# Meng-333/SRADSGAN

Hardware: AMD Instinct MI355X
Metric: training images/sec (216x216, x4) (higher is better)
Workload: dtype f32 (split-bf16 products: 3 bf16 MFMA terms per fp32 multiply, fp32 accumulate)

## Files before the change

sradsgan_amd/csrc/conv_api.hip:

```cpp
#include "conv_internal.h"
#include "conv_dev.h"

using namespace srhip;

namespace srhip {
struct PackEntry {
  const float* w;
  float* packed;
  int cout, cin, kh, kw, mode, fast;
};
__global__ __launch_bounds__(256) void pack_batched_kernel(const PackEntry* __restrict__ tab) {
  const PackEntry e = tab[blockIdx.y];
  const int khkw = e.kh * e.kw;
  if (e.fast) {
    constexpr int LDS_F = 32 * (16 * 9 + 1);
    __shared__ float tile[LDS_F];
    const long total = (long)e.cout * e.cin * khkw;
    const int RO = e.mode == 0 ? 8 : 32;
    const int CI = e.mode == 0 ? (khkw <= 9 ? 64 : 16) : (khkw <= 9 ? 16 : 4);
    const int ld = CI * khkw + 1;
    const int nci = (e.cin + CI - 1) / CI, nco = (e.cout + RO - 1) / RO;
    const int ndst = e.mode == 0 ? e.cout : e.cin, csrc = e.mode == 0 ? e.cin : e.cout;
    const long ndst16 = ((long)ndst + 15) / 16 * 16;
    float* s0 = e.packed;
// ... 5 lines not shown
      const int cw = min(CI, e.cin - ci0), rw = min(RO, e.cout - co0);
      const int rowlen = cw * khkw;
      __syncthreads();
      for (int i = threadIdx.x; i < rw * rowlen; i += 256) {
        const int r = i / rowlen, k = i - r * rowlen;
        tile[r * ld + k] = e.w[((size_t)(co0 + r) * e.cin + ci0) * khkw + k];
      }
      __syncthreads();
      auto at = [&](int a, int b, int tap) { return tile[a * ld + b * khkw + tap]; };
      const int nn = e.mode == 0 ? rw : cw, nc = e.mode == 0 ? cw : rw;
      const int n0 = e.mode == 0 ? co0 : ci0, c00 = e.mode == 0 ? ci0 : co0;
      for (int it = threadIdx.x; it < nn * khkw * (nc / 8); it += 256) {
        const int g8 = it % (nc / 8), rt = it / (nc / 8);
        const int tap = rt % khkw, dn = rt / khkw;
        float v[8];
#pragma unroll
        for (int j = 0; j < 8; ++j) v[j] = e.mode == 0 ? at(dn, g8 * 8 + j, tap) : at(g8 * 8 + j, dn, tap);
        const long idx = ((long)(n0 + dn) * khkw + tap) * csrc + c00 + g8 * 8;
        reinterpret_cast<float4*>(s0 + idx)[0] = make_float4(v[0], v[1], v[2], v[3]);
        reinterpret_cast<float4*>(s0 + idx)[1] = make_float4(v[4], v[5], v[6], v[7]);
        bf16x8_t hi, lo;
        split_bf16x8(make_float4(v[0], v[1], v[2], v[3]), make_float4(v[4], v[5], v[6], v[7]), hi, lo);
        *reinterpret_cast<u32x4*>(s1 + idx * 4) = __builtin_bit_cast(u32x4, hi);
        *reinterpret_cast<u32x4*>(s1 + idx * 4 + 16) = __builtin_bit_cast(u32x4, lo);
        const f16x8_t f16 = {(_Float16)v[0], (_Float16)v[1], (_Float16)v[2], (_Float16)v[3], (_Float16)v[4], (_Float16)v[5], (_Float16)v[6], (_Float16)v[7]};
        const u32x4 z = {0u, 0u, 0u, 0u};
        *reinterpret_cast<u32x4*>(s2 + idx * 4) = __builtin_bit_cast(u32x4, f16);
        *reinterpret_cast<u32x4*>(s2 + idx * 4 + 16) = z;
      }
      for (int it = threadIdx.x; it < nn * khkw * (nc / 16); it += 256) {
        const int dn = it % nn, rt = it / nn;
        const int tap = rt % khkw, g16 = rt / khkw;
        const int n = n0 + dn, swz = (n >> 2) & 3;
        char* row = s3 + (((long)((c00 >> 4) + g16) * khkw + tap) * ndst16 + n) * 64;
#pragma unroll
        for (int h = 0; h < 2; ++h) {
          float v[8];
#pragma unroll
          for (int j = 0; j < 8; ++j) v[j] = e.mode == 0 ? at(dn, g16 * 16 + h * 8 + j, tap) : at(g16 * 16 + h * 8 + j, dn, tap);
          bf16x8_t hi, lo;
          split_bf16x8(make_float4(v[0], v[1], v[2], v[3]), make_float4(v[4], v[5], v[6], v[7]), hi, lo);
          *reinterpret_cast<u32x4*>(row + (((2 * h) ^ swz) << 4)) = __builtin_bit_cast(u32x4, hi);
          *reinterpret_cast<u32x4*>(row + (((2 * h + 1) ^ swz) << 4)) = __builtin_bit_cast(u32x4, lo);
        }
      }
    }
  } else {
    const int csrc = e.mode == 0 ? e.cin : e.cout, cdst = e.mode == 0 ? e.cout : e.cin;
    const int ld = ((cdst + 31) / 32) * 32;
    const long total = (long)khkw * csrc * ld;
    for (long idx = (long)blockIdx.x * blockDim.x + threadIdx.x; idx < total; idx += (long)gridDim.x * blockDim.x) {
      const int row = (int)(idx / ld), col = (int)(idx - (long)row * ld);
      float v = 0.f;
      if (col < cdst) {
        const int tap = row / csrc, cs = row - tap * csrc;
        const int a = tap / e.kw, b = tap - a * e.kw;
        if (e.mode == 0)
          v = e.w[(((size_t)col * e.cin + cs) * e.kh + a) * e.kw + b];
        else
          v = e.w[(((size_t)cs * e.cin + col) * e.kh + (e.kh - 1 - a)) * e.kw + (e.kw - 1 - b)];
      }
      e.packed[idx] = v;
    }
  }
}
}

namespace srhip {
extern int g_fast_cfg;
extern int g_wgrad_cfg;
extern int g_rowtap_addr;
extern int g_rowtap_pipe;
extern int g_patch_ks;
extern int g_fast_dynlds;
extern int g_fast_ablate;
extern int g_conv_math;
extern int g_sgam_cfg;
extern int g_pers_grid;
extern int g_pers_small;
extern int g_pool_epi_any;
extern int g_pers_abl;
extern int g_phase_batch;
extern int g_headconv_rows;
}
extern int g_tail_dbg;
namespace srhip {
}

namespace srhip {
struct Probe {
  int kind = 0, n = 0, h = 0, w = 0, cin = 0, cout = 0, cap = 0, count = 0;
  hipEvent_t ev[2 * 1024];
  int units[1024];
  int created = 0;
};
static Probe g_probe;
static inline bool probe_hit(int kind, int n, int h, int w, int cin, int cout) {
  return g_probe.kind == kind && g_probe.count < g_probe.cap && g_probe.n == n && g_probe.h == h && g_probe.w == w && g_probe.cin == cin &&
         g_probe.cout == cout;
}
static inline int probe_begin(void* stream) {
  const int i = g_probe.count;
  (void)hipEventRecord(g_probe.ev[2 * i], as_stream(stream));
  return i;
}
static inline void probe_end(int i, void* stream, int units = 1) {
  (void)hipEventRecord(g_probe.ev[2 * i + 1], as_stream(stream));
  g_probe.units[i] = units;
  g_probe.count = i + 1;
}
}

extern "C" {

int srhip_probe_config(int kind, int n, int h, int w, int cin, int cout, int max_pairs) {
  SRHIP_REQUIRE(kind >= 0 && kind <= 3 && max_pairs >= 0 && max_pairs <= 1024, "probe_config: kind 0..3, max_pairs <= 1024");
  while (g_probe.created < 2 * max_pairs) {
    if (hipEventCreate(&g_probe.ev[g_probe.created]) != hipSuccess) {
      set_error("probe_config: hipEventCreate failed");
      return SRHIP_ERR_LAUNCH;
    }
    ++g_probe.created;
  }
  g_probe.kind = kind; g_probe.n = n; g_probe.h = h; g_probe.w = w; g_probe.cin = cin; g_probe.cout = cout;
  g_probe.cap = kind ? max_pairs : 0;
  g_probe.count = 0;
  return SRHIP_OK;
}
int srhip_probe_read(float* ms, int* units, int cap) {
  SRHIP_REQUIRE(ms || cap == 0, "probe_read: null buffer");
  const int n = g_probe.count < cap ? g_probe.count : cap;
  for (int i = 0; i < n; ++i) {
    if (hipEventSynchronize(g_probe.ev[2 * i + 1]) != hipSuccess || hipEventElapsedTime(&ms[i], g_probe.ev[2 * i], g_probe.ev[2 * i + 1]) != hipSuccess) {
      set_error("probe_read: event %d not readable", i);
      return -1;
    }
    if (units) units[i] = g_probe.units[i];
  }
  return n;
}

int srhip_debug_set(int key, int value) {
  if (key == 0) {
    g_fast_cfg = value;
    return SRHIP_OK;
  }
  if (key == 1) {
    g_wgrad_cfg = value;
    return SRHIP_OK;
  }
  if (key == 2) {
    g_fast_dynlds = value;
    return SRHIP_OK;
  }
  if (key == 3) {
    g_fast_ablate = value;
    return SRHIP_OK;
  }
  if (key == 4) {
    g_sgam_cfg = value;
    return SRHIP_OK;
  }
  if (key == 5) {
    g_pers_grid = value;
    return SRHIP_OK;
  }
  if (key == 6) {
    g_pers_abl = value;
    return SRHIP_OK;
  }
  if (key == 7) {
    g_tail_dbg = value;
    return SRHIP_OK;
  }
  if (key == 8) {
    g_rowtap_addr = value;
    return SRHIP_OK;
  }
  if (key == 9) {
    g_rowtap_pipe = value;
    return SRHIP_OK;
  }
  if (key == 10) {
    g_patch_ks = value;
    return SRHIP_OK;
  }
  if (key == 11) {
    g_pers_small = value;
    return SRHIP_OK;
  }
  if (key == 12) {
    g_flat_blocks = value > 0 ? value : 768;
    return SRHIP_OK;
  }
  if (key == 13) {
    g_flat_abl = value;
    return SRHIP_OK;
  }
  if (key == 14) {
    g_flat_f32_k8 = value;
    return SRHIP_OK;
  }
  if (key == 15) {
    g_patch8 = value;
    return SRHIP_OK;
  }
  if (key == 16) {
    g_patch8_abl = value;
    return SRHIP_OK;
  }
  if (key == 17) {
    g_phase_batch = value;
    return SRHIP_OK;
  }
  if (key == 18) {
    g_headconv_rows = value;
    return SRHIP_OK;
  }
  if (key == 19) {
    g_pool_epi_any = value;
    return SRHIP_OK;
  }
  return SRHIP_ERR_ARG;
}

int srhip_set_conv_math(int mode) {
  SRHIP_REQUIRE(mode == SRHIP_MATH_FP32 || mode == SRHIP_MATH_BF16X3 || mode == SRHIP_MATH_HALF, "set_conv_math: unknown mode");
  g_conv_math = mode;
  return SRHIP_OK;
}
int srhip_get_conv_math(void) { return g_conv_math; }

size_t srhip_packed_elems(int cout, int cin, int kh, int kw, int mode) {
  if (cout <= 0 || cin <= 0 || kh <= 0 || kw <= 0 || (mode != 0 && mode != 1)) return 0;
  const bool fast = mode == 0 ? fast_fwd_ok(cin, cout, kh, kw) : fast_dgrad_ok(cin, cout, kh, kw);
  if (fast)
    return 3 * (size_t)cout * cin * kh * kw + (size_t)fast_tiled_elems(mode == 0 ? cout : cin, mode == 0 ? cin : cout, kh * kw);
  const int csrc = mode == 0 ? cin : cout, cdst = mode == 0 ? cout : cin;
  return (size_t)kh * kw * csrc * legacy_packed_ld(cdst);
}

int srhip_pack_entry_bytes(void) { return (int)sizeof(PackEntry); }

int srhip_packed_is_fast(int cout, int cin, int kh, int kw, int mode) {
  return (mode == 0 ? fast_fwd_ok(cin, cout, kh, kw) : fast_dgrad_ok(cin, cout, kh, kw)) ? 1 : 0;
}

int srhip_pack_weights_batched(const void* entries_dev, int count, void* stream) {
  SRHIP_REQUIRE(entries_dev && count >= 0, "pack_weights_batched: bad argument");
  if (count == 0) return SRHIP_OK;
  hipLaunchKernelGGL(pack_batched_kernel, dim3(32, count), dim3(256), 0, as_stream(stream),
                     static_cast<const PackEntry*>(entries_dev));
  return check_launch("pack_weights_batched");
}

int srhip_pack_weight(const float* w, float* packed, int cout, int cin, int kh, int kw, int mode, void* stream) {
  SRHIP_REQUIRE(w && packed && cout > 0 && cin > 0 && kh > 0 && kw > 0 && (mode == 0 || mode == 1),
                "pack_weight: bad argument");
  const bool fast = mode == 0 ? fast_fwd_ok(cin, cout, kh, kw) : fast_dgrad_ok(cin, cout, kh, kw);
  if (fast) return fast_pack_weight(w, packed, cout, cin, kh, kw, mode, as_stream(stream));
  return legacy_pack_weight(w, packed, cout, cin, kh, kw, mode, stream);
}

int srhip_conv2d_fwd(const float* x, const float* packed, const float* bias, const float* residual,
                     const float* rowscale, const float* chanscale, float* y, int n, int h, int w, int cin, int cout, int kh, int kw,
                     int stride, int pad, int ldx, int ldy, int ldr, float slope, int flags, void* stream) {
  SRHIP_REQUIRE(x && packed && y, "conv2d_fwd: null tensor");
  SRHIP_REQUIRE(n >= 0 && h > 0 && w > 0 && cin > 0 && cout > 0 && kh > 0 && kw > 0 && stride > 0 && pad >= 0,
                "conv2d_fwd: bad geometry");
  SRHIP_REQUIRE(ldx >= cin && ldy >= cout, "conv2d_fwd: row stride smaller than channel count");
  SRHIP_REQUIRE(!(flags & SRHIP_EPI_BIAS) || bias, "conv2d_fwd: EPI_BIAS without bias");
  SRHIP_REQUIRE(!(flags & SRHIP_EPI_RESIDUAL) || (residual && ldr >= cout), "conv2d_fwd: EPI_RESIDUAL without residual");
  SRHIP_REQUIRE(!(flags & SRHIP_EPI_ROWSCALE) || rowscale, "conv2d_fwd: EPI_ROWSCALE without rowscale");
  SRHIP_REQUIRE(!(flags & SRHIP_EPI_CHANSCALE) || chanscale, "conv2d_fwd: EPI_CHANSCALE without chanscale");
  if (fast_fwd_ok(cin, cout, kh, kw)) {
    const bool pr = probe_hit(1, n, h, w, cin, cout);
    const int pi = pr ? probe_begin(stream) : 0;
    const int rc = fast_conv2d_fwd(x, packed, bias, residual, rowscale, chanscale, y, n, h, w, cin, cout, kh, kw, stride, pad, ldx, ldy,
                                   ldr, slope, flags, as_stream(stream));
    if (pr) probe_end(pi, stream);
    return rc;
  }
  SRHIP_REQUIRE(!(flags & SRHIP_EPI_CHANSCALE), "conv2d_fwd: EPI_CHANSCALE needs Cin % 16 == 0");
  return legacy_conv2d_fwd(x, packed, bias, residual, rowscale, y, n, h, w, cin, cout, kh, kw, stride, pad, ldx, ldy,
                           ldr, slope, flags, stream);
}

int srhip_conv2d_fwd_dual(const float* x, const float* packed, const float* bias, const float* residual, const float* rowscale,
                          const float* chanscale, float* y, void* y_pp, int* served, int n, int h, int w, int cin, int cout, int kh,
                          int kw, int stride, int pad, int ldx, int ldy, int ldr, float slope, int flags, void* stream) {
  SRHIP_REQUIRE(y_pp && served && (((uintptr_t)y_pp) & 15) == 0 && ldy == cout, "conv2d_fwd_dual: 16-byte aligned plane buffer, dense fp32 output");
  g_dst2_req.pp = y_pp;
  g_dst2_req.served = 0;
  const int rc = srhip_conv2d_fwd(x, packed, bias, residual, rowscale, chanscale, y, n, h, w, cin, cout, kh, kw, stride, pad, ldx, ldy, ldr,
                                  slope, flags, stream);
  *served = g_dst2_req.served;
  g_dst2_req.pp = nullptr;
  g_dst2_req.served = 0;
  return rc;
}

int srhip_conv2d_fwd_pool(const float* x, const float* packed, const float* bias, float* y, float* pool, size_t pool_sec_bytes,
                          int* nseg_out, int n, int h, int w, int cin, int cout, int ldx, int ldy, int flags, void* stream) {
// ... 279 lines not shown
```

sradsgan_amd/csrc/conv_fast.hip:

```cpp
#include "conv_dev.h"

namespace srhip {

int g_fast_ablate = 0;



template <int BM, int BN, int WM, int WN, int BK, int MATH = 0>
__global__ __launch_bounds__(WM* WN * 64) void fast_conv_kernel(const float* __restrict__ src,
                                                                 const float* __restrict__ wt,
                                                                 const float* __restrict__ bias,
                                                                 const float* __restrict__ residual,
                                                                 const float* __restrict__ rowscale,
                                                                 const float* __restrict__ chanscale,
                                                                 const float* __restrict__ actmask,
                                                                 float* __restrict__ dst, FastGeom g, int nblk_m,
                                                                 int nblk_n) {
  constexpr int NT = WM * WN * 64;
  constexpr int WTM = BM / WM, WTN = BN / WN;
  constexpr int TM = WTM / 32, TN = WTN / 32;
  constexpr int LS = BK + 4;
  constexpr int QPR = BK / 4;
  constexpr int RPP = NT / QPR;
  constexpr int AR = (BM + RPP - 1) / RPP, BR = (BN + RPP - 1) / RPP;
// ... 1067 lines not shown
template <int ND>
__global__ __launch_bounds__(256) void narrow_conv_kernel(const float* __restrict__ src, const float* __restrict__ wt,
                                                           const float* __restrict__ bias, float* __restrict__ dst,
                                                           FastGeom g, int tiles_h, int tiles_w, int lo_h, int lo_w) {
  constexpr int PW = 16, PH = 16, PWP = PW + 2, PR = (PH + 2) * PWP;
  __shared__ __attribute__((aligned(16))) float4 lds[2][PR * 4];
  const int tid = threadIdx.x;
  const int tpi = tiles_h * tiles_w;
  const int img = blockIdx.x / tpi;
  const int prem = blockIdx.x - img * tpi;
  const int ty = prem / tiles_w, tx = prem - ty * tiles_w;
  const int oh0 = ty * PH, ow0 = tx * PW;
  const int py = tid >> 4, px = tid & 15;

  int soff[6];
  int sdst[6];
#pragma unroll
  for (int i = 0; i < 6; ++i) {
    const int e = tid + i * 256;
    soff[i] = -1;
    sdst[i] = 0;
    if (e < PR * 4) {
      const int row = e >> 2, q = e & 3;
      const int pi = row / PWP, pj = row - pi * PWP;
      const int sh = oh0 + lo_h + pi, sw = ow0 + lo_w + pj;
      sdst[i] = row * 4 + (q ^ (row & 3));
      if (sh >= 0 && sh < g.Hs && sw >= 0 && sw < g.Ws) soff[i] = ((img * g.Hs + sh) * g.Ws + sw) * g.lds + q * 4;
      else soff[i] = -2;
    }
  }
  const int CC = g.C / 16;
  float4 stage[6];
  auto fetch = [&](int cc) {
#pragma unroll
    for (int i = 0; i < 6; ++i)
      stage[i] = soff[i] >= 0 ? *reinterpret_cast<const float4*>(src + (size_t)soff[i] + cc * 16) : make_float4(0.f, 0.f, 0.f, 0.f);
  };
  auto commit = [&](int buf) {
#pragma unroll
    for (int i = 0; i < 6; ++i)
      if (soff[i] != -1) lds[buf][sdst[i]] = stage[i];
  };
  float acc[ND];
#pragma unroll
  for (int n = 0; n < ND; ++n) acc[n] = 0.f;

  fetch(0);
  commit(0);
  __syncthreads();
  for (int cc = 0; cc < CC; ++cc) {
    const int buf = cc & 1;
    if (cc + 1 < CC) fetch(cc + 1);
#pragma unroll 1
    for (int tap = 0; tap < 9; ++tap) {
      {
        const int th = tap / 3, tw = tap - th * 3;
        const int a_th = (g.dh0 + th * g.dhs) - lo_h, a_tw = (g.dw0 + tw * g.dws) - lo_w;
        const int row = (py + a_th) * PWP + px + a_tw;
        const int wk = ((g.kh0 + th * g.khs) * g.KW + (g.kw0 + tw * g.kws)) * g.C + cc * 16;
#pragma unroll
        for (int q = 0; q < 4; ++q) {
          const float4 v = lds[buf][row * 4 + (q ^ (row & 3))];
#pragma unroll
          for (int n = 0; n < ND; ++n) {
            const float* w = wt + (size_t)n * g.ldw + wk + q * 4;
            acc[n] = fmaf(v.x, w[0], acc[n]);
            acc[n] = fmaf(v.y, w[1], acc[n]);
            acc[n] = fmaf(v.z, w[2], acc[n]);
            acc[n] = fmaf(v.w, w[3], acc[n]);
          }
        }
      }
    }
    if (cc + 1 < CC) commit(buf ^ 1);
    __syncthreads();
  }
  const int oh = oh0 + py, ow = ow0 + px;
  if (oh < g.OH && ow < g.OW) {
    const size_t dpix = ((size_t)img * g.Hd + oh) * g.Wd + ow;
#pragma unroll
    for (int n = 0; n < ND; ++n) {
      if (n < g.K) {
        float v = acc[n];
        if (g.flags & SRHIP_EPI_BIAS) v += bias[n];
        if (g.flags & SRHIP_EPI_LRELU) v = v > 0.f ? v : v * g.slope;
        dst[dpix * g.ldd + n] = v;
      }
    }
  }
}

struct WgradGeom {
  int N, H, W, C, ldx;
  int Ho, Wo, K, ldy;
  int KH, KW, stride, pad;
  int P;
  int Ktot;
  int nsplit, chunks_per_split;
  unsigned x_bytes, dy_bytes;
};

template <int BM, int BN, int WM, int WN>
__global__ __launch_bounds__(256) void fast_wgrad_kernel(const float* __restrict__ x, const float* __restrict__ dy,
                                                          float* __restrict__ partial,
                                                          float* __restrict__ bias_partial,
                                                          const float* __restrict__ xrow,
                                                          const float* __restrict__ xchan, WgradGeom g) {
  constexpr int WTM = BM / WM, WTN = BN / WN;
  constexpr int TM = WTM / 32, TN = WTN / 32;
  constexpr int LDA = BM + 4, LDB = BN + 4;
  constexpr int AV = (FBK * BM / 4) / 256, BV = (FBK * BN / 4) / 256;
  static_assert(AV >= 1 && BV >= 1, "tile too small");
  constexpr int STAGE = FBK * (LDA + LDB);
  __shared__ __attribute__((aligned(16))) float lds[2 * STAGE];

  const int tid = threadIdx.x;
  const int ntn = (g.Ktot + BN - 1) / BN;
  const int ntm = (g.K + BM - 1) / BM;
  int tile_n, tile_m, split;
  {
    const int tps = ntm * ntn;
    int bid = blockIdx.x;
    if (g.nsplit % 8 == 0) {
      const int j = bid >> 3;
      split = (j / tps) * 8 + (bid & 7);
      bid = j % tps;
    } else {
      split = bid / tps;
      bid -= split * tps;
    }
    tile_n = bid % ntn;
    tile_m = bid / ntn;
  }
  const int m0 = tile_m * BM, n0 = tile_n * BN;

  __amdgpu_buffer_rsrc_t rx = __builtin_amdgcn_make_buffer_rsrc(const_cast<float*>(x), 0, g.x_bytes, 0x00020000);
  __amdgpu_buffer_rsrc_t ry = __builtin_amdgcn_make_buffer_rsrc(const_cast<float*>(dy), 0, g.dy_bytes, 0x00020000);

  const int c_begin = split * g.chunks_per_split;
  const int nchunks_total = (g.P + FBK - 1) / FBK;
  const int c_end = min(c_begin + g.chunks_per_split, nchunks_total);

  constexpr int AQ = BM / 4, BQ = BN / 4;
  const int a_row0 = tid / AQ, a_c = tid - a_row0 * AQ;
  const int b_row0 = tid / BQ, b_c = tid - b_row0 * BQ;
  const bool a_colok = (m0 + a_c * 4) < g.K;
  const int kcol = n0 + b_c * 4;
  const bool b_colok = kcol < g.Ktot;
  const int tap = kcol / g.C, ci0 = kcol - tap * g.C;
  const int kh = tap / g.KW, kw = tap - kh * g.KW;

  int bn[BV], bho[BV], bwo[BV];
#pragma unroll
  for (int j = 0; j < BV; ++j) {
    const int p = c_begin * FBK + b_row0 + j * (256 / BQ);
    const int HoWo = g.Ho * g.Wo;
    bn[j] = p / HoWo;
    const int rem = p - bn[j] * HoWo;
    bho[j] = rem / g.Wo;
    bwo[j] = rem - bho[j] * g.Wo;
  }

  float4 ra[AV], rb[BV], rxs[BV];
  float4 bsum = make_float4(0.f, 0.f, 0.f, 0.f);
  const bool xscale = xrow != nullptr || xchan != nullptr;
  auto load_tiles = [&](int kc) {
// ... 958 lines not shown
                                 int kw, int mode) {
  const int idx = blockIdx.x * blockDim.x + threadIdx.x;
  const int total = cout * cin * kh * kw;
  if (idx >= total) return;
  const int khkw = kh * kw;
  if (mode == 0) {
    const int co = idx / (khkw * cin);
    const int rem = idx - co * khkw * cin;
    const int tap = rem / cin, ci = rem - tap * cin;
    fast_pack_store(packed, total, idx, w[((size_t)co * cin + ci) * khkw + tap], cout, cin, khkw);
  } else {
    const int ci = idx / (khkw * cout);
    const int rem = idx - ci * khkw * cout;
    const int tap = rem / cout, co = rem - tap * cout;
    fast_pack_store(packed, total, idx, w[((size_t)co * cin + ci) * khkw + tap], cin, cout, khkw);
  }
}

static bool shape_ok(int csrc, int kh, int kw) { return csrc % 16 == 0 && kh * kw <= 32 && kh == kw; }
bool fast_fwd_ok(int cin, int cout, int kh, int kw) { return shape_ok(cin, kh, kw); }
bool fast_dgrad_ok(int cin, int cout, int kh, int kw) { return shape_ok(cout, kh, kw); }
bool fast_wgrad_ok(int cin, int cout, int kh, int kw) { return cin % 16 == 0 && cout % 4 == 0 && kh == kw; }

int fast_pack_weight(const float* w, float* packed, int cout, int cin, int kh, int kw, int mode, hipStream_t st) {
  const long total = (long)cout * cin * kh * kw;
  hipLaunchKernelGGL(fast_pack_kernel, dim3(cdiv(total, 256)), dim3(256), 0, st, w, packed, cout, cin, kh, kw, mode);
  return check_launch("fast_pack_weight");
}

thread_local Dst2Request g_dst2_req;
thread_local ResRequest g_res_req;
thread_local PhaseRequest g_phase_req;
int g_conv_math = 0;
int g_fast_dynlds = 0;
template <int BM, int BN, int WM, int WN, int BK>
static int launch_fast(const float* src, const float* wt, const float* bias, const float* residual,
                       const float* rowscale, const float* chanscale, const float* actmask, float* dst,
                       const FastGeom& g, hipStream_t st) {
  const int nbm = cdiv(g.M, BM), nbn = cdiv(g.K, BN);
  hipLaunchKernelGGL((fast_conv_kernel<BM, BN, WM, WN, BK>), dim3(nbm * nbn), dim3(WM * WN * 64), g_fast_dynlds, st, src, wt, bias,
                     residual, rowscale, chanscale, actmask, dst, g, nbm, nbn);
  return check_launch("fast_conv");
}

__global__ __launch_bounds__(256) void dot_conv_kernel(const float* __restrict__ src, const float* __restrict__ wt,
                                                        const float* __restrict__ bias, float* __restrict__ dst, FastGeom g) {
  const int lane = threadIdx.x & 63;
  const int m = blockIdx.x * 4 + (threadIdx.x >> 6);
  if (m >= g.M) return;
  const int ow = m % g.OW, t = m / g.OW;
  const int oh = t % g.OH, n = t / g.OH;
  float acc = 0.f;
  for (int th = 0; th < g.TH; ++th) {
    const int sh = oh * g.ss + g.dh0 + th * g.dhs;
    if (sh < 0 || sh >= g.Hs) continue;
    for (int tw = 0; tw < g.TW; ++tw) {
      const int sw = ow * g.ss + g.dw0 + tw * g.dws;
      if (sw < 0 || sw >= g.Ws) continue;
      const float* xp = src + ((size_t)(n * g.Hs + sh) * g.Ws + sw) * g.lds;
      const float* wp = wt + (size_t)((g.kh0 + th * g.khs) * g.KW + (g.kw0 + tw * g.kws)) * g.C;
      for (int c = lane * 4; c < g.C; c += 256) {
        const float4 a = *reinterpret_cast<const float4*>(xp + c);
        const float4 b = *reinterpret_cast<const float4*>(wp + c);
        acc = fmaf(a.x, b.x, acc);
        acc = fmaf(a.y, b.y, acc);
        acc = fmaf(a.z, b.z, acc);
        acc = fmaf(a.w, b.w, acc);
      }
    }
  }
#pragma unroll
  for (int o = 32; o >= 1; o >>= 1) acc += __shfl_xor(acc, o, 64);
  if (lane == 0) {
    float v = acc;
    if (g.flags & SRHIP_EPI_BIAS) v += bias[0];
    if (g.flags & SRHIP_EPI_LRELU) v = v > 0.f ? v : v * g.slope;
    dst[((size_t)(n * g.Hd + oh * g.dsd + g.ph) * g.Wd + ow * g.dsd + g.pw) * g.ldd] = v;
  }
}

int g_patch_ks = 1;
int g_fast_cfg = 0;
int g_phase_batch = 1;

static bool plan_patch(const FastGeom& g, PatchGeom* pg, double min_eff = 0.70) {
  if (g.TH != 3 || g.TW != 3 || g.ss != 1 || g.dsd != 1 || g.ph != 0 || g.pw != 0) return false;
  if ((g.dhs != 1 && g.dhs != -1) || (g.dws != 1 && g.dws != -1)) return false;
  if (g.Hd != g.OH || g.Wd != g.OW) return false;
  double best = 0.0;
  for (int pw = 4; pw <= 64 && pw <= g.OW + 3; ++pw) {
    int ph = 128 / pw;
    if (ph > g.OH) ph = g.OH;
    if (ph < 1 || (ph + 2) * (pw + 2) > 192) continue;
    const long tiles = (long)cdiv(g.OH, ph) * cdiv(g.OW, pw);
    const double eff = (double)g.OH * g.OW / ((double)tiles * 128.0) + 1e-6 * (double)(pw - pw % 16) / pw;
    if (eff > best + 1e-9) {
      best = eff;
      pg->PH = ph; pg->PW = pw;
    }
  }
  if (best < min_eff || best <= 0.0) return false;
  pg->tiles_h = cdiv(g.OH, pg->PH);
  pg->tiles_w = cdiv(g.OW, pg->PW);
  pg->PWP = pg->PW + 2;
  pg->PR = (pg->PH + 2) * pg->PWP;
  pg->npieces = cdiv(pg->PR, 16);
  pg->lo_h = g.dhs > 0 ? g.dh0 : g.dh0 + 2 * g.dhs;
  pg->lo_w = g.dws > 0 ? g.dw0 : g.dw0 + 2 * g.dws;
  const int a = pg->PW >> 4;
  const int nfull = pg->PH * a < 8 ? pg->PH * a : 8;
  auto base = [&](int q) { return ((q / a) * pg->PWP + (q % a) * 16) & 15; };
  int fin[8], nf = 0, singles[8], ns = 0;
  bool used[8] = {false, false, false, false, false, false, false, false};
  for (int q = 0; q < nfull; ++q) {
    if (used[q]) continue;
    used[q] = true;
    int partner = -1;
    for (int p2 = q + 1; p2 < nfull; ++p2)
      if (!used[p2] && base(p2) == base(q)) {
        partner = p2;
        break;
      }
    if (partner >= 0) {
      used[partner] = true;
      fin[nf++] = q;
      fin[nf++] = partner;
    } else {
      singles[ns++] = q;
    }
  }
  for (int i = 0; i < ns; ++i) fin[nf++] = singles[i];
  for (int q = nfull; q < 8; ++q) fin[nf++] = q;
  pg->gmap = 0;
  for (int i = 0; i < 8; ++i) pg->gmap |= (unsigned)(fin[i] & 15) << (4 * i);
  return true;
}

long pp_sign_tiles(int n, int h, int w, int cout) {
  if (cout < 128 || cout % 128 != 0) return 0;
  FastGeom g;
  g.TH = 3; g.TW = 3; g.ss = 1; g.dsd = 1; g.ph = 0; g.pw = 0; g.dhs = 1; g.dws = 1; g.dh0 = -1; g.dw0 = -1;
  g.Hd = g.OH = h; g.Wd = g.OW = w;
  PatchGeom pg;
  if (!plan_patch(g, &pg, 0.0)) return 0;
  return (long)n * pg.tiles_h * pg.tiles_w * (cout / 128);
}

static int run_fast(const float* src, const float* wt, const float* bias, const float* residual,
                    const float* rowscale, const float* chanscale, const float* actmask, float* dst, const FastGeom& g,
                    hipStream_t st) {
  if (g.M <= 0) return SRHIP_OK;
  if (g.src_pp || g.dst_pp) {
    PatchGeom pg;
    const int ef = g.flags & 0x3f;
    if (g_conv_math == 1 && g.K >= 64 && g.K % 8 == 0 && g.C % 32 == 0 && !(ef & (SRHIP_EPI_CHANSCALE | SRHIP_EPI_ROWSCALE)) && !g.accumulate &&
        plan_patch(g, &pg, 0.0)) {
      const int nbm = g.N * pg.tiles_h * pg.tiles_w;
      const bool wide = g.K >= 128;
      const int nbn = cdiv(g.K, wide ? 128 : 64);
      if (wide && !residual) {
        const int rc8 = launch_patch8(src, wt, bias, actmask, dst, g, pg, nbm, ef, st);
        if (rc8 >= 0) return rc8;
      }
      const int rc = launch_patch_pers(src, wt, bias, residual, actmask, dst, g, pg, nbm, nbn, wide, 0, ef, st);
      if (rc >= 0) return rc;
    }
    set_error("conv2d (padded planes): shape / arithmetic mode not served by the persistent patch kernel");
    return SRHIP_ERR_ARG;
  }
#define SRHIP_LF(BM_, BN_, WM_, WN_, BK_) \
  return launch_fast<BM_, BN_, WM_, WN_, BK_>(src, wt, bias, residual, rowscale, chanscale, actmask, dst, g, st)
  if (g.K <= 4 && g_fast_cfg != 20 && g_fast_cfg != 22 && g.TH == 3 && g.TW == 3 && g.ss == 1 && g.dsd == 1 && g.ph == 0 &&
      g.pw == 0 && g.Hd == g.OH && g.Wd == g.OW && (g.dhs == 1 || g.dhs == -1) && (g.dws == 1 || g.dws == -1) &&
      !(g.flags & ~(SRHIP_EPI_BIAS | SRHIP_EPI_LRELU | SRHIP_EPI_GRADDATA)) && !g.accumulate && g.M >= 65536) {
    const int th = cdiv(g.OH, 16), tw = cdiv(g.OW, 16);
    const int lo_h = g.dhs > 0 ? g.dh0 : g.dh0 + 2 * g.dhs, lo_w = g.dws > 0 ? g.dw0 : g.dw0 + 2 * g.dws;
    if (g.K == 3)
      hipLaunchKernelGGL((narrow_conv_kernel<3>), dim3(g.N * th * tw), dim3(256), 0, st, src, wt, bias, dst, g, th, tw, lo_h, lo_w);
    else
      hipLaunchKernelGGL((narrow_conv_kernel<4>), dim3(g.N * th * tw), dim3(256), 0, st, src, wt, bias, dst, g, th, tw, lo_h, lo_w);
    return check_launch("narrow_conv");
  }
  if (g.K == 1 && g.C % 4 == 0 && g.lds % 4 == 0 && (((uintptr_t)src | (uintptr_t)wt) & 15) == 0 && g.M < 65536 && g_fast_cfg != 20 &&
      g_fast_cfg != 22 && !(g.flags & ~(SRHIP_EPI_BIAS | SRHIP_EPI_LRELU | SRHIP_EPI_GRADDATA)) && !g.accumulate) {
    hipLaunchKernelGGL(dot_conv_kernel, dim3(cdiv(g.M, 4)), dim3(256), 0, st, src, wt, bias, dst, g);
    return check_launch("dot_conv");
  }
  const int prod = g_conv_math == 2 ? ((g.flags & SRHIP_EPI_GRADDATA) ? 1 : 2) : 0;
  const float* w16 = wt + (size_t)(g.w_bytes >> 2) * (prod == 2 ? 2 : 1);
  if (g.K <= 32 && g_conv_math >= 1 && g_fast_cfg != 20 && !(g.flags & (SRHIP_EPI_CHANSCALE | 0x300))) {
    const int nbm = cdiv(g.M, 128), nbn = cdiv(g.K, 32);
    if (prod == 0)
      hipLaunchKernelGGL((fast_conv_kernel<128, 32, 4, 1, 16, 1>), dim3(nbm * nbn), dim3(256), g_fast_dynlds, st, src,
                         w16, bias, residual, rowscale, chanscale, actmask, dst, g, nbm, nbn);
    else if (prod == 1)
      hipLaunchKernelGGL((fast_conv_kernel<128, 32, 4, 1, 16, 2>), dim3(nbm * nbn), dim3(256), g_fast_dynlds, st, src,
                         w16, bias, residual, rowscale, chanscale, actmask, dst, g, nbm, nbn);
    else
      hipLaunchKernelGGL((fast_conv_kernel<128, 32, 4, 1, 16, 3>), dim3(nbm * nbn), dim3(256), g_fast_dynlds, st, src,
                         w16, bias, residual, rowscale, chanscale, actmask, dst, g, nbm, nbn);
    return check_launch("fast_conv");
  }
  if (g.K <= 32) SRHIP_LF(128, 32, 4, 1, 16);
  const int eflags = g.flags & 0x3f;
  const bool al16 = g.K % 4 == 0 && g.ldd % 4 == 0 && ((uintptr_t)dst & 15) == 0 && (!residual || (g.ldr % 4 == 0 && ((uintptr_t)residual & 15) == 0)) &&
                    (!actmask || ((uintptr_t)actmask & 15) == 0) && (!bias || ((uintptr_t)bias & 15) == 0);
  bool patch_to_dma = false;
  if (g_conv_math >= 1 && g_fast_cfg != 20 && g_fast_cfg != 21 && (g_fast_cfg < 1 || g_fast_cfg == 23 || g_fast_cfg == 24) && !(g.flags & 0x300) && g.K >= 64 && al16 &&
      !(eflags & (SRHIP_EPI_CHANSCALE | SRHIP_EPI_ROWSCALE)) && !g.accumulate) {
    PatchGeom pg;
    if (plan_patch(g, &pg)) {
      const int nbm = g.N * pg.tiles_h * pg.tiles_w;
      const bool wide = g.K >= 128 && g_fast_cfg != 24;
      const int nbn = cdiv(g.K, wide ? 128 : 64);
      if (g_fast_cfg == 23) {
        patch_to_dma = (long)nbm * nbn >= 256;
      } else if ((long)nbm * nbn >= 256 || g_fast_cfg == -2) {
        const float* wsplit = w16;
        if (!(g.flags & 0x400) && wide && prod == 0 && !residual && g_fast_cfg != 23) {
          const int rc8 = launch_patch8(src, wt, bias, actmask, dst, g, pg, nbm, eflags, st);
          if (rc8 >= 0) return rc8;
        }
        if (!(g.flags & 0x400)) {
          const int rc = launch_patch_pers(src, wt, bias, residual, actmask, dst, g, pg, nbm, nbn, wide, prod, eflags, st);
          if (rc >= 0) return rc;
        }
        if (prod != 0) {
#define SRHIP_LPH(BN_, PROD_)                                                                                       \
  do {                                                                                                              \
    hipLaunchKernelGGL((conv_patch_kernel<BN_, -1, PROD_>), dim3(nbm * nbn), dim3(256), 0, st, src, wsplit, bias,   \
                       residual, actmask, dst, g, pg, nbm, nbn);                                                   \
    return check_launch("conv_patch");                                                                              \
  } while (0)
          if (wide && prod == 1) SRHIP_LPH(128, 1);
          if (wide) SRHIP_LPH(128, 2);
          if (prod == 1) SRHIP_LPH(64, 1);
          SRHIP_LPH(64, 2);
#undef SRHIP_LPH
        }
#define SRHIP_LP(BN_, EPI_)                                                                                         \
  do {                                                                                                              \
    hipLaunchKernelGGL((conv_patch_kernel<BN_, EPI_>), dim3(nbm * nbn), dim3(256), 0, st, src, wsplit, bias,       \
                       residual, actmask, dst, g, pg, nbm, nbn);                                                   \
    return check_launch("conv_patch");                                                                              \
  } while (0)
#define SRHIP_LPE(BN_)                                                  \
  do {                                                                  \
    if (eflags == 0) SRHIP_LP(BN_, 0);                                  \
    if (eflags == SRHIP_EPI_BIAS) SRHIP_LP(BN_, 1);                     \
    if (eflags == (SRHIP_EPI_BIAS | SRHIP_EPI_LRELU)) SRHIP_LP(BN_, 3); \
    if (eflags == SRHIP_EPI_ACTMASK) SRHIP_LP(BN_, 32);                 \
    if (eflags == SRHIP_EPI_RESIDUAL) SRHIP_LP(BN_, 4);                 \
    SRHIP_LP(BN_, -1);                                                  \
  } while (0)
        if (wide) SRHIP_LPE(128);
        if (g_patch_ks && g.C % 32 == 0 && g.C >= 32) {
#define SRHIP_LK(EPI_)                                                                                              \
  do {                                                                                                              \
    hipLaunchKernelGGL((conv_patch_ks_kernel<EPI_>), dim3(nbm * nbn), dim3(256), 0, st, src, wsplit, bias, residual, \
// ... 544 lines not shown
```

sradsgan_amd/ops.py:

```python
import contextlib
import ctypes
import os
import threading
import weakref

import torch
from torch.autograd import Function

from . import _hip

EPI_BIAS, EPI_LRELU, EPI_RESIDUAL, EPI_ROWSCALE, EPI_CHANSCALE, EPI_GRADDATA = 1, 2, 4, 8, 16, 64
CL = torch.channels_last

class _State:
    skip_param_grads = False
    direct_grads = False
    wgrad_stream = None
    skip_ids = frozenset()
    stop_ids = frozenset()
    capturing = False
    wgrad_group = 1
    pending = None
    held = None
    last_out_pp = None
# ... 561 lines not shown
    cout, cin = dw0.shape[0], dw0.shape[1]
    n, _, h, wd = x0.shape
    lib = _hip.lib()
    xpp, ypp = int(isinstance(x0, PP)), int(isinstance(dy0, PP))
    for it in items[1:]:
        if int(isinstance(it[0], PP)) != xpp or int(isinstance(it[1], PP)) != ypp:
            raise RuntimeError('conv2d_wgrad_pp: the convolutions of one launch must share their operand formats (planes / fp32)')
    mask = lib.srhip_conv2d_wgrad_pp_ok(n, h, wd, cin, cout)
    want = 4 if (xpp and ypp) else 1 if ypp else 2 if xpp else 0
    if not (mask & want):
        raise RuntimeError('conv2d_wgrad_pp: shape %s -> %d not served with these operand formats (served mask %d)' % (tuple(x0.shape), cout, mask))
    k = len(items)
    tab = ctypes.c_void_p * k
    xs = tab(*[it[0].data_ptr() for it in items])
    dys = tab(*[it[1].data_ptr() for it in items])
    dws = tab(*[it[2].data_ptr() for it in items])
    dbs = tab(*[(it[3].data_ptr() if it[3] is not None else None) for it in items])
    nbytes = lib.srhip_conv2d_wgrad_pp_workspace(k, xpp, ypp, n, h, wd, cin, cout)
    if on_stream is not None:
        ws = _side_workspace(nbytes, dw0.device, on_stream)
        st = ctypes.c_void_p(on_stream.cuda_stream)
    else:
        ws = torch.empty((max(nbytes, 4) + 3) // 4, device=dw0.device, dtype=torch.float32)
        st = _stream()
    _hip.check(lib.srhip_conv2d_wgrad_pp(k, xs, dys, xpp, ypp, dws, dbs, 1 if accumulate else 0, _p(ws), ws.numel() * 4, n, h, wd, cin, cout,
                                        cout if xpp else cin, st), 'conv2d_wgrad_pp')


class _PlanePool:

    def __init__(self):
        self.free = {}
        self.created = 0

    def get(self, n, c, h, w, device):
        key = (n, c, h, w, device.index)
        q = self.free.get(key)
        capturing = _state.capturing or torch.cuda.is_current_stream_capturing()
        if capturing:
            key = key + ('capture',)
            q = self.free.get(key)
        if q:
            for i, (pp, evs) in enumerate(q):
                if capturing:
                    del q[i]
                    cur = torch.cuda.current_stream()
                    for st in evs:
                        if st != cur:
                            cur.wait_stream(st)
                    return pp
                if all(ev.query() for ev in evs):
                    del q[i]
                    return pp
        self.created += 1
        return pp_empty(n, c, h, w, device)

    def release_all(self):
        for key, q in self.free.items():
            for pp, evs in q:
                for ev in evs:
                    ev.synchronize()
        self.free.clear()

    def begin_capture(self):
        for key in [k for k in self.free if k[-1] == 'capture']:
            del self.free[key]

    def put(self, pp, streams=()):
        capturing = _state.capturing or torch.cuda.is_current_stream_capturing()
        evs = list(streams) if capturing else [s.record_event() for s in streams]
        key = (pp.n, pp.c, pp.h, pp.w, pp.buf.device.index) + (('capture',) if capturing else ())
        self.free.setdefault(key, []).append((pp, evs))


plane_pool = _PlanePool()
if os.environ.get('SRHIP_PERS_GRID'):
    _hip.lib().srhip_debug_set(5, int(os.environ['SRHIP_PERS_GRID']))
if os.environ.get('SRHIP_FLAT_BLOCKS'):
    _hip.lib().srhip_debug_set(12, int(os.environ['SRHIP_FLAT_BLOCKS']))
if os.environ.get('SRHIP_POOL_EPI_ANY'):
    _hip.lib().srhip_debug_set(19, int(os.environ['SRHIP_POOL_EPI_ANY']))
if os.environ.get('SRHIP_FLAT_F32_K8'):
    _hip.lib().srhip_debug_set(14, int(os.environ['SRHIP_FLAT_F32_K8']))
if os.environ.get('SRHIP_TAIL_DBG'):
    _hip.lib().srhip_debug_set(7, int(os.environ['SRHIP_TAIL_DBG']))
_X_PP = os.environ.get('SRHIP_X_PP', '1') == '1'
_DU_PP = os.environ.get('SRHIP_DU_PP', '1') == '1'
_PP_RAB = os.environ.get('SRHIP_PP_RAB', '1') == '1'
_PP_SIGNS = os.environ.get('SRHIP_PP_SIGNS', '1') == '1'


def rab_planes_ok(x, w1, w2):
    if not (_PP_RAB and x.is_cuda and get_conv_math() == 'bf16x3'):
        return False
    n, c, h, w = x.shape
    cm = w1.shape[0]
    lib = _hip.lib()
    return (tuple(w1.shape[2:]) == (3, 3) and tuple(w2.shape[2:]) == (3, 3) and w2.shape[0] == c and w2.shape[1] == cm
            and bool(lib.srhip_conv2d_pp_ok(n, h, w, c, cm)) and bool(lib.srhip_conv2d_pp_ok(n, h, w, cm, c))
            and (lib.srhip_conv2d_wgrad_pp_ok(n, h, w, c, cm) & 4) and (lib.srhip_conv2d_wgrad_pp_ok(n, h, w, cm, c) & 4))


_WGRAD_PP_CONVERT = os.environ.get('SRHIP_WGRAD_PP_CONVERT', '1') == '1'


def _to_planes(t, device):
    n, c, h, w = t.shape
    pp = plane_pool.get(n, c, h, w, device)
    return pp_from_f32(t, out=pp)


def _launch_wgrad_pp(items, side):
    main = torch.cuda.current_stream()
    run_on = side if side is not None else main
    with torch.cuda.stream(run_on):
        conv = []
        launch = []
        for x, dy, gw, gb, release in items:
            xo, dyo = x, dy
            if _WGRAD_PP_CONVERT:
                if not isinstance(x, PP):
                    xo = _to_planes(x, gw.device)
                    conv.append(xo)
                if not isinstance(dy, PP):
                    dyo = _to_planes(dy, gw.device)
                    conv.append(dyo)
            launch.append((xo, dyo, gw, gb))
        conv2d_wgrad_pp_raw(launch, accumulate=True, on_stream=side)
        for pp in conv:
            plane_pool.put(pp, (run_on,))
        for x, dy, gw, gb, release in items:
            for pp in release:
                plane_pool.put(pp, (run_on,) if side is None else (run_on, main))
    if side is not None:
        for x, dy, gw, gb, release in items:
            for t in (x, dy):
                if not isinstance(t, PP):
                    t.record_stream(side)
            if not isinstance(dy, PP):
                _hold_for_side(side, dy)


def wgrad_pp_for_params(w, b, x, dy, want_b, release=()):
    gw = _grad_slot(w)
    gb = _grad_slot(b) if (want_b and b is not None) else None
    if gw is None or (want_b and b is not None and gb is None):
        return False
    side = _state.wgrad_stream
    _age_pending()
    item = (x, dy, gw, gb, tuple(release))
    if side is None:
        _launch_wgrad_pp([item], None)
        return True
    if _state.wgrad_group > 1:
        key = ('pp', tuple(x.shape), w.shape[0], gb is not None, isinstance(x, PP), isinstance(dy, PP))
        q = _state.pending.setdefault(key, [])
        q.append(item + (_stream().value, _state.wgrad_seq))
        if len(q) >= _PP_GROUP:
            if _WGRAD_SLOTS and _state.ready_pairs is not None and not _state.capturing:
                _state.ready_pairs.append(_state.pending.pop(key))
            else:
                _flush_key(key)
        return True
    _fork_side(side)
    _launch_wgrad_pp([item], side)
    return True
# ... 1513 lines not shown
```

Measured before the change: 669.4.

## Add MFMA-based narrow-output conv kernel for 64-channel inputs

Adds a new kernel for 3x3 convolutions with few output channels (K<=4) and 64 input channels. For every pixel in a 18x18 halo patch it computes all 9 tap partial products with fp32 MFMA 16x16x4 instructions, writes them to LDS, then sums the taps per output pixel. This replaces the scalar FMA narrow_conv path for large-M cases, moving the channel reduction onto matrix cores. The cost is redundant halo work and a large LDS footprint (up to 324x37 floats), which may limit occupancy.

```diff
diff --git a/sradsgan_amd/csrc/conv_api.hip b/sradsgan_amd/csrc/conv_api.hip
--- a/sradsgan_amd/csrc/conv_api.hip
+++ b/sradsgan_amd/csrc/conv_api.hip
@@ -111,6 +111,7 @@
 extern int g_pers_abl;
 extern int g_phase_batch;
 extern int g_headconv_rows;
+extern int g_narrow_mfma;
 }
 extern int g_tail_dbg;
 namespace srhip {
@@ -248,6 +249,10 @@
   }
   if (key == 19) {
     g_pool_epi_any = value;
+    return SRHIP_OK;
+  }
+  if (key == 20) {
+    g_narrow_mfma = value;
     return SRHIP_OK;
   }
   return SRHIP_ERR_ARG;
diff --git a/sradsgan_amd/csrc/conv_fast.hip b/sradsgan_amd/csrc/conv_fast.hip
--- a/sradsgan_amd/csrc/conv_fast.hip
+++ b/sradsgan_amd/csrc/conv_fast.hip
@@ -1173,6 +1173,110 @@
     for (int n = 0; n < ND; ++n) {
       if (n < g.K) {
         float v = acc[n];
+        if (g.flags & SRHIP_EPI_BIAS) v += bias[n];
+        if (g.flags & SRHIP_EPI_LRELU) v = v > 0.f ? v : v * g.slope;
+        dst[dpix * g.ldd + n] = v;
+      }
+    }
+  }
+}
+
+template <int ND>
+__global__ __launch_bounds__(256) void narrow_mfma_kernel(const float* __restrict__ src, const float* __restrict__ wt,
+                                                          const float* __restrict__ bias, float* __restrict__ dst,
+                                                          FastGeom g, int tiles_h, int tiles_w, int lo_h, int lo_w) {
+  constexpr int PW = 16, PH = 16, PWP = PW + 2, PR = (PH + 2) * PWP;
+  constexpr int NC = 9 * ND, NT = (NC + 15) / 16;
+  constexpr int ZS = NC | 1;
+  constexpr int MT = (PR + 15) / 16, TPW = (MT + 3) / 4;
+  __shared__ float zl[PR * ZS];
+  const int tid = threadIdx.x, lane = tid & 63, wave = __builtin_amdgcn_readfirstlane(tid >> 6);
+  const int m = lane & 15, q = lane >> 4;
+  const int tpi = tiles_h * tiles_w;
+  const int img = blockIdx.x / tpi;
+  const int prem = blockIdx.x - img * tpi;
+  const int ty = prem / tiles_w, tx = prem - ty * tiles_w;
+  const int oh0 = ty * PH, ow0 = tx * PW;
+
+  float bw[NT][2][8];
+#pragma unroll
+  for (int nt = 0; nt < NT; ++nt) {
+    const int col = min(nt * 16 + m, NC - 1);
+    const int tap = col / ND, co = col - tap * ND;
+    const int th = tap / 3, tw = tap - th * 3;
+    const float* w = wt + co * g.ldw + ((g.kh0 + th * g.khs) * g.KW + (g.kw0 + tw * g.kws)) * 64 + 8 * q;
+#pragma unroll
+    for (int c = 0; c < 2; ++c)
+#pragma unroll
+      for (int i = 0; i < 8; ++i) bw[nt][c][i] = w[32 * c + i];
+  }
+  auto in_image = [&](int r, int* sh, int* sw) {
+    const int pi = r / PWP, pj = r - pi * PWP;
+    *sh = oh0 + lo_h + pi;
+    *sw = ow0 + lo_w + pj;
+    return r < PR && *sh >= 0 && *sh < g.Hs && *sw >= 0 && *sw < g.Ws;
+  };
+  float4 a[TPW][4];
+  auto fetch = [&](int t) {
+    int sh, sw;
+    in_image(min((wave + 4 * t) * 16 + m, PR - 1), &sh, &sw);
+    sh = min(max(sh, 0), g.Hs - 1);
+    sw = min(max(sw, 0), g.Ws - 1);
+    const float* p = src + ((size_t)(img * g.Hs + sh) * g.Ws + sw) * g.lds + 8 * q;
+#pragma unroll
+    for (int h = 0; h < 4; ++h) a[t][h] = *reinterpret_cast<const float4*>(p + 32 * (h >> 1) + 4 * (h & 1));
+  };
+  fetch(0);
+  fetch(1);
+#pragma unroll
+  for (int t = 0; t < TPW; ++t) {
+    if (wave + 4 * t >= MT) break;
+    if (t + 2 < TPW) fetch(t + 2);
+    f32x4 acc[NT];
+#pragma unroll
+    for (int nt = 0; nt < NT; ++nt) acc[nt] = f32x4{0.f, 0.f, 0.f, 0.f};
+#pragma unroll
+    for (int c = 0; c < 2; ++c)
+#pragma unroll
+      for (int i = 0; i < 8; ++i) {
+        const float4 v = a[t][2 * c + (i >> 2)];
+        const float av = (i & 3) == 0 ? v.x : (i & 3) == 1 ? v.y : (i & 3) == 2 ? v.z : v.w;
+#pragma unroll
+        for (int nt = 0; nt < NT; ++nt) acc[nt] = __builtin_amdgcn_mfma_f32_16x16x4f32(av, bw[nt][c][i], acc[nt], 0, 0, 0);
+      }
+#pragma unroll
+    for (int r = 0; r < 4; ++r) {
+      const int row = (wave + 4 * t) * 16 + 4 * q + r;
+      int sh, sw;
+      const bool inside = in_image(row, &sh, &sw);
+#pragma unroll
+      for (int nt = 0; nt < NT; ++nt) {
+        const int col = nt * 16 + m;
+        if (row < PR && col < NC) zl[row * ZS + col] = inside ? acc[nt][r] : 0.f;
+      }
+    }
+  }
+  __syncthreads();
+
+  const int py = tid >> 4, px = tid & 15;
+  const int oh = oh0 + py, ow = ow0 + px;
+  if (oh < g.OH && ow < g.OW) {
+    float o[ND];
+#pragma unroll
+    for (int n = 0; n < ND; ++n) o[n] = 0.f;
+#pragma unroll
+    for (int tap = 0; tap < 9; ++tap) {
+      const int th = tap / 3, tw = tap - th * 3;
+      const int a_th = (g.dh0 + th * g.dhs) - lo_h, a_tw = (g.dw0 + tw * g.dws) - lo_w;
+      const int row = (py + a_th) * PWP + px + a_tw;
+#pragma unroll
+      for (int n = 0; n < ND; ++n) o[n] += zl[row * ZS + tap * ND + n];
+    }
+    const size_t dpix = ((size_t)img * g.Hd + oh) * g.Wd + ow;
+#pragma unroll
+    for (int n = 0; n < ND; ++n) {
+      if (n < g.K) {
+        float v = o[n];
         if (g.flags & SRHIP_EPI_BIAS) v += bias[n];
         if (g.flags & SRHIP_EPI_LRELU) v = v > 0.f ? v : v * g.slope;
         dst[dpix * g.ldd + n] = v;
@@ -2297,6 +2401,7 @@
 int g_patch_ks = 1;
 int g_fast_cfg = 0;
 int g_phase_batch = 1;
+int g_narrow_mfma = 1;
 
 static bool plan_patch(const FastGeom& g, PatchGeom* pg, double min_eff = 0.70) {
   if (g.TH != 3 || g.TW != 3 || g.ss != 1 || g.dsd != 1 || g.ph != 0 || g.pw != 0) return false;
@@ -2390,6 +2495,15 @@
       !(g.flags & ~(SRHIP_EPI_BIAS | SRHIP_EPI_LRELU | SRHIP_EPI_GRADDATA)) && !g.accumulate && g.M >= 65536) {
     const int th = cdiv(g.OH, 16), tw = cdiv(g.OW, 16);
     const int lo_h = g.dhs > 0 ? g.dh0 : g.dh0 + 2 * g.dhs, lo_w = g.dws > 0 ? g.dw0 : g.dw0 + 2 * g.dws;
+    if (g_narrow_mfma && g.C == 64 && g.lds % 4 == 0 && ((uintptr_t)src & 15) == 0) {
+#define SRHIP_NM(ND_) hipLaunchKernelGGL((narrow_mfma_kernel<ND_>), dim3(g.N * th * tw), dim3(256), 0, st, src, wt, bias, dst, g, th, tw, lo_h, lo_w)
+      if (g.K == 1) SRHIP_NM(1);
+      else if (g.K == 2) SRHIP_NM(2);
+      else if (g.K == 3) SRHIP_NM(3);
+      else SRHIP_NM(4);
+#undef SRHIP_NM
+      return check_launch("narrow_mfma");
+    }
     if (g.K == 3)
       hipLaunchKernelGGL((narrow_conv_kernel<3>), dim3(g.N * th * tw), dim3(256), 0, st, src, wt, bias, dst, g, th, tw, lo_h, lo_w);
     else
diff --git a/sradsgan_amd/ops.py b/sradsgan_amd/ops.py
--- a/sradsgan_amd/ops.py
+++ b/sradsgan_amd/ops.py
@@ -667,6 +667,8 @@
     _hip.lib().srhip_debug_set(19, int(os.environ['SRHIP_POOL_EPI_ANY']))
 if os.environ.get('SRHIP_FLAT_F32_K8'):
     _hip.lib().srhip_debug_set(14, int(os.environ['SRHIP_FLAT_F32_K8']))
+if os.environ.get('SRHIP_NARROW_MFMA'):
+    _hip.lib().srhip_debug_set(20, int(os.environ['SRHIP_NARROW_MFMA']))
 if os.environ.get('SRHIP_TAIL_DBG'):
     _hip.lib().srhip_debug_set(7, int(os.environ['SRHIP_TAIL_DBG']))
 _X_PP = os.environ.get('SRHIP_X_PP', '1') == '1'
```

New measurement: 673.8, median of 6. About the same (+0.7%).
